# husheng876/pytorch_nested-unet

Hardware: AMD Instinct MI355X
Metric: images/sec NestedUNet 96x96 bs=16 train (higher is better)
Workload: dtype bf16; 1 GPU; NestedUNet(num_classes=1, in=3, deep_supervision=False) 96x96 per-GPU batch 16, bf16 storage / fp32 accumulate, BCEDiceLoss, SGD(1e-3, 0.9, wd 1e-4), fwd+loss+iou+bwd+sgd per step (BASELINE.json configs[1]); global_batch=16, parallelism=dp1, hip_graph=True

## Files before the change

### include/nunet.h

```cpp
#ifndef NUNET_H
#define NUNET_H

#include <stddef.h>
#include <stdint.h>

#ifdef __cplusplus
extern "C" {
#endif

typedef void* nunet_stream_t;

enum { NUNET_F32 = 0, NUNET_BF16 = 1, NUNET_F16 = 2 };
enum {
  NUNET_OK = 0,
  NUNET_EINVAL = -1,
  NUNET_ELAUNCH = -2,
  NUNET_ENODEV = -3
};

int nunet_version(void);
const char* nunet_last_error(void);

#define NUNET_BN_SUM_REPLICAS 8
#define NUNET_FX_WORDS 2
// ... 260 lines not shown
int nunet_plan_grad_scratch(const nunet_plan* p, int64_t* byte_offset, int64_t* bucket0_floats,
                            int64_t* total_floats);
int nunet_plan_bucket0_wait(nunet_plan* p, nunet_stream_t s);
int nunet_plan_opt_step(nunet_plan* p, float* params, const nunet_optim* opt, void* arena, size_t arena_bytes, float grad_scale,
                        float* grads, nunet_stream_t s);
size_t nunet_plan_grad_sqnorm_ws_bytes(const nunet_plan* p);
int nunet_plan_grad_sqnorm(nunet_plan* p, const void* arena, size_t arena_bytes, double* ws, size_t ws_bytes, nunet_stream_t s);
int nunet_plan_repack(nunet_plan* p, const float* params, void* arena, size_t arena_bytes, nunet_stream_t s);
int nunet_plan_set_multistream(nunet_plan* p, int32_t enable);
enum { NUNET_SCHEDULE_LANES = 0, NUNET_SCHEDULE_LIST = 2 };
int nunet_plan_calibrate(nunet_plan* p, int32_t begin);
int nunet_plan_set_lane_priority(nunet_plan* p, int32_t lowest);
int nunet_plan_reset_lanes(nunet_plan* p);
int nunet_plan_set_schedule(nunet_plan* p, int32_t schedule);
int nunet_plan_set_wgrad_dy(nunet_plan* p, int32_t in_loader);
int64_t nunet_plan_feature(const nunet_plan* p, int32_t i, int32_t j, int32_t* pitch,
                           int32_t* channels);

typedef struct {
  char name[48];
  int32_t launches;
  double ms, flops, bytes;
} nunet_prof_entry;
int nunet_profile_begin(void);
int nunet_profile_end(nunet_prof_entry* out, int32_t max_entries, int32_t* n_out);
typedef struct nunet_graph nunet_graph;
int nunet_graph_begin(nunet_stream_t stream);
int nunet_graph_end(nunet_stream_t stream, nunet_graph** out);
int nunet_graph_launch(nunet_graph* graph, nunet_stream_t stream);
int nunet_graph_info(const nunet_graph* graph, int32_t* nodes, int32_t* edges, int32_t* lanes);
// ... 15 lines not shown
```

### pytorch_nested-unet_amd/_lib.py

```python
import ctypes as C
import os
import subprocess

import torch

_HERE = os.path.dirname(os.path.abspath(__file__))
LIB_PATH = os.environ.get("NUNET_LIB_PATH") or os.path.join(_HERE, "libnunet.so")

F32, BF16, F16 = 0, 1, 2
DTYPES = {"fp32": F32, "float32": F32, "bf16": BF16, "bfloat16": BF16, "fp16": F16, "float16": F16,
          torch.float32: F32, torch.bfloat16: BF16, torch.float16: F16}
TORCH_DTYPE = {F32: torch.float32, BF16: torch.bfloat16, F16: torch.float16}

_vp, _i32, _i64, _u32, _f32, _sz = C.c_void_p, C.c_int32, C.c_int64, C.c_uint32, C.c_float, C.c_size_t
BN_SUM_REPLICAS = 8
FX_WORDS = 2
TF_NONE, TF_BN_RELU, TF_BN_RELU_BWD = 0, 1, 2


def fx_zeros(c, device):
    return torch.zeros(BN_SUM_REPLICAS * 2 * c * FX_WORDS, dtype=torch.int64, device=device)


def fx_decode(buf, c):
# ... 212 lines not shown
    "nunet_plan_backward_phase": (_i32, [_vp, _vp, _vp, _vp, _sz, _vp, _i32, _i32, _vp]),
    "nunet_plan_grad_scratch": (_i32, [_vp, C.POINTER(_i64), C.POINTER(_i64), C.POINTER(_i64)]),
    "nunet_plan_bucket0_wait": (_i32, [_vp, _vp]),
    "nunet_plan_opt_step": (_i32, [_vp, _vp, C.POINTER(Optim), _vp, _sz, _f32, _vp, _vp]),
    "nunet_plan_grad_sqnorm_ws_bytes": (C.c_size_t, [_vp]),
    "nunet_plan_grad_sqnorm": (_i32, [_vp, _vp, _sz, _vp, _sz, _vp]),
    "nunet_plan_repack": (_i32, [_vp, _vp, _vp, _sz, _vp]),
    "nunet_plan_feature": (_i64, [_vp, _i32, _i32, C.POINTER(_i32), C.POINTER(_i32)]),
    "nunet_plan_feature_grad": (_i64, [_vp, _i32, _i32, C.POINTER(_i32), C.POINTER(_i32)]),
    "nunet_plan_block_act1": (_i32, [_vp, _vp, _vp, _sz, _i32, _i32, _vp, _vp]),
    "nunet_plan_census_count": (_i32, [_vp, _i32]),
    "nunet_plan_census_get": (_i32, [_vp, _i32, _i32, C.POINTER(PlanCensusEntry)]),
    "nunet_plan_set_multistream": (_i32, [_vp, _i32]),
    "nunet_plan_set_schedule": (_i32, [_vp, _i32]),
    "nunet_plan_set_wgrad_dy": (_i32, [_vp, _i32]),
    "nunet_plan_calibrate": (_i32, [_vp, _i32]),
    "nunet_plan_set_lane_priority": (_i32, [_vp, _i32]),
    "nunet_plan_reset_lanes": (_i32, [_vp]),
    "nunet_plan_set_lanes": (_i32, [_vp, C.POINTER(_vp), _i32]),
    "nunet_profile_begin": (_i32, []),
    "nunet_profile_end": (_i32, [C.POINTER(ProfEntry), _i32, C.POINTER(_i32)]),
    "nunet_debug_spin": (_i32, [_i32, _i32, _vp]),
    "nunet_debug_stamp": (_i32, [_vp, _vp]),
    "nunet_conv3x3_launch_info": (_i32, [C.POINTER(ConvDesc), C.POINTER(ConvLaunchInfo)]),
    "nunet_conv3x3_wgrad_launch_info": (_i32, [C.POINTER(WgradDesc), C.POINTER(WgradLaunchInfo)]),
    "nunet_conv_kernel_attrs": (_i32, [C.POINTER(ConvDesc), C.POINTER(ConvKernelAttrs)]),
    "nunet_loss_launch_info": (_i32, [_i32, _i32, _i64, _i32, C.POINTER(LossLaunchInfo)]),
    "nunet_graph_begin": (_i32, [_vp]),
    "nunet_graph_end": (_i32, [_vp, C.POINTER(_vp)]),
    "nunet_graph_launch": (_i32, [_vp, _vp]),
# ... 84 lines not shown
```

### pytorch_nested-unet_amd/csrc/common.h

```cpp
#pragma once
#include <hip/hip_runtime.h>
#include <hip/hip_ext.h>
#include <stdint.h>
#include <stdio.h>
#include <stdarg.h>
#include <string.h>
#include <type_traits>

#include "../../include/nunet.h"
#include "../../include/nunet_diag.h"

typedef __bf16 bf16_t;
typedef _Float16 f16_t;

typedef __attribute__((ext_vector_type(4))) float f32x4;
typedef __attribute__((ext_vector_type(16))) float f32x16;
typedef __attribute__((ext_vector_type(8))) __bf16 bf16x8;
typedef __attribute__((ext_vector_type(8))) _Float16 f16x8;
typedef __attribute__((ext_vector_type(4))) short s16x4;
typedef __attribute__((ext_vector_type(4))) uint32_t u32x4;

#define WAVE 64
#define CONV_GROUP_MAX 4

// ... 32 lines not shown
    if (pe0_) hipExtLaunchKernelGGL(kernel, grid, block, shmem, stream, pe0_, pe1_, 0, __VA_ARGS__);            \
    else hipLaunchKernelGGL(kernel, grid, block, shmem, stream, __VA_ARGS__);                                   \
  } while (0)

int nunet_zero_async(void* p, size_t bytes, hipStream_t st);

bool seg_active();
bool seg_wait(hipStream_t st, hipEvent_t ev);
bool seg_record(hipEvent_t ev, hipStream_t st);
void seg_touch(hipStream_t st);

static inline int dtype_size(int dt) { return dt == NUNET_F32 ? 4 : 2; }
static inline int ceil_div(int a, int b) { return (a + b - 1) / b; }
static inline int64_t ceil_div64(int64_t a, int64_t b) { return (a + b - 1) / b; }
static inline size_t align_up(size_t a, size_t b) { return (a + b - 1) / b * b; }

template <typename T> struct Tr;
template <> struct Tr<float> {
  static constexpr int EPV = 4;
  static constexpr int DT = NUNET_F32;
};
template <> struct Tr<bf16_t> {
  static constexpr int EPV = 8;
  static constexpr int DT = NUNET_BF16;
};
template <> struct Tr<f16_t> {
  static constexpr int EPV = 8;
  static constexpr int DT = NUNET_F16;
};

// ... 166 lines not shown
  A = __builtin_fmaf(-B, mean, sc * k1);
}

template <typename T> __device__ __forceinline__ Vec16<T> ld16(const T* p) {
  Vec16<T> v;
  v.raw = *reinterpret_cast<const u32x4*>(p);
  return v;
}
template <typename T> __device__ __forceinline__ void st16(T* p, const Vec16<T>& v) {
  *reinterpret_cast<u32x4*>(p) = v.raw;
}
template <typename T> __device__ __forceinline__ Vec16<T> zero16() {
  Vec16<T> v;
  v.raw = u32x4{0u, 0u, 0u, 0u};
  return v;
}

__device__ __forceinline__ float wave_sum(float v) {
#pragma unroll
  for (int o = 32; o > 0; o >>= 1) v += __shfl_xor(v, o);
  return v;
}

__device__ __forceinline__ double wave_sum_f64(double v) {
#pragma unroll
  for (int o = 32; o > 0; o >>= 1) v += __shfl_xor(v, o);
  return v;
}
__device__ __forceinline__ double block256_sum_f64(double v, double* s_w4) {
  v = wave_sum_f64(v);
// ... 99 lines not shown
```

### pytorch_nested-unet_amd/csrc/elementwise.hip

```cpp
#include <cmath>
#include <stdlib.h>
#include <string.h>

#include "common.h"

static thread_local char g_err[512] = "";
void nunet_set_error(const char* fmt, ...) {
  va_list ap;
  va_start(ap, fmt);
  vsnprintf(g_err, sizeof(g_err), fmt, ap);
  va_end(ap);
}
int nunet_check_launch(const char* what) {
  hipError_t e = hipGetLastError();
  if (e != hipSuccess) {
    nunet_set_error("%s: launch failed: %s", what, hipGetErrorString(e));
    return NUNET_ELAUNCH;
  }
  static int trace = -1;
  if (trace < 0) { const char* t = getenv("NUNET_TRACE_LAUNCH"); trace = t ? atoi(t) : 0; }
  if (trace) {
    fprintf(stderr, "[nunet] %s ... ", what); fflush(stderr);
    e = hipDeviceSynchronize();
    fprintf(stderr, "%s\n", e == hipSuccess ? "ok" : hipGetErrorString(e)); fflush(stderr);
    if (e != hipSuccess) { nunet_set_error("%s: execution failed: %s", what, hipGetErrorString(e)); return NUNET_ELAUNCH; }
  }
  return NUNET_OK;
}
extern "C" const char* nunet_last_error(void) { return g_err; }
extern "C" int nunet_version(void) { return 104; }

static inline int grid_for(int64_t items, int block, int cap = 256 * 16) {
  int64_t g = ceil_div64(items, block);
  if (g > cap) g = cap;
  if (g < 1) g = 1;
  return (int)g;
}

__global__ __launch_bounds__(256) void zero_kernel(u32x4* __restrict__ p16, size_t n16, uint32_t* __restrict__ tail, int ntail) {
  const u32x4 z = {0u, 0u, 0u, 0u};
  for (size_t i = blockIdx.x * (size_t)blockDim.x + threadIdx.x; i < n16; i += (size_t)gridDim.x * blockDim.x) p16[i] = z;
  if (blockIdx.x == 0 && (int)threadIdx.x < ntail) tail[threadIdx.x] = 0u;
}
int nunet_zero_async(void* p, size_t bytes, hipStream_t st) {
  NUNET_REQUIRE(((uintptr_t)p % 16) == 0 && bytes % 4 == 0, "zero: buffer must be 16-byte aligned, size a multiple of 4");
  const size_t n16 = bytes / 16;
  const int ntail = (int)((bytes % 16) / 4);
  NUNET_LAUNCH(zero_kernel, dim3(grid_for((int64_t)n16, 256 * 4, 2048)), dim3(256), 0, st, (u32x4*)p, n16,
                     (uint32_t*)((char*)p + n16 * 16), ntail);
  return nunet_check_launch("zero");
}

template <typename T>
__global__ __launch_bounds__(256) void nchw_to_nhwc_kernel(const float* __restrict__ x, int C, int hw, T* __restrict__ y, int cpad, int gshift) {
  constexpr int EPV = Tr<T>::EPV;
  const int n = blockIdx.y;
  const int groups = 1 << gshift;
  const float* xi = x + (size_t)n * C * hw;
  T* yi = y + (size_t)n * hw * cpad;
  for (int j = blockIdx.x * blockDim.x + threadIdx.x; j < (hw << gshift); j += gridDim.x * blockDim.x) {
    const int pix = j >> gshift, c0 = (j & (groups - 1)) * EPV;
    Vec16<T> v;
#pragma unroll
    for (int e = 0; e < EPV; ++e) v.set(e, c0 + e < C ? xi[(size_t)(c0 + e) * hw + pix] : 0.f);
    st16(yi + (size_t)pix * cpad + c0, v);
  }
}
template <typename T> static int launch_nchw_to_nhwc(const float* x, int N, int C, int H, int W, void* y, int cpad, hipStream_t st) {
  constexpr int EPV = Tr<T>::EPV;
  const int groups = cpad / EPV;
  int gshift = 0;
  while ((1 << gshift) < groups) ++gshift;
  NUNET_REQUIRE(cpad % EPV == 0 && (1 << gshift) == groups && N <= 65535, "nchw_to_nhwc: cpad=%d must be a power-of-two number of 16-byte groups", cpad);
  const long long hw = (long long)H * W;
  NUNET_REQUIRE(hw * groups < (1ll << 31), "nchw_to_nhwc: image too large");
  const int64_t total = (int64_t)N * H * W * cpad;
  ProfScope ps(PC_LAYOUT, 0, (double)total * sizeof(T) + (double)N * C * H * W * 4, st);
  NUNET_LAUNCH((nchw_to_nhwc_kernel<T>), dim3(grid_for(hw * groups, 256, 1024), N), dim3(256), 0, st, x, C, (int)hw, (T*)y, cpad, gshift);
  return nunet_check_launch("nchw_to_nhwc");
}
extern "C" int nunet_nchw_to_nhwc(const float* x, int32_t N, int32_t C, int32_t H, int32_t W, int32_t dtype, void* y, int32_t cpad, nunet_stream_t s) {
  NUNET_REQUIRE(x && y && N > 0 && C > 0 && H > 0 && W > 0 && cpad >= C, "nchw_to_nhwc: bad args");
  return NUNET_DISPATCH(dtype, launch_nchw_to_nhwc, x, N, C, H, W, y, cpad, (hipStream_t)s);
}

__global__ __launch_bounds__(256) void preprocess_u8_kernel(const uint8_t* __restrict__ u, int N, int H, int W, int C,
                                                             const float* __restrict__ mean, const float* __restrict__ stdv,
                                                             const int32_t* __restrict__ aug, float post_scale, float* __restrict__ out) {
  const int64_t total = (int64_t)N * C * H * W;
  for (int64_t i = blockIdx.x * (int64_t)blockDim.x + threadIdx.x; i < total; i += (int64_t)gridDim.x * blockDim.x) {
    const int x = (int)(i % W);
    int64_t t = i / W;
    const int y = (int)(t % H); t /= H;
// ... 1881 lines not shown
```

### pytorch_nested-unet_amd/csrc/plan.hip

```cpp
#include <stdlib.h>
#include <string.h>

#include <initializer_list>
#include <functional>
#include <algorithm>

#include <map>
#include <string>
#include <vector>
#include <stdarg.h>

#include "common.h"

static const int NBF[5] = {32, 64, 128, 256, 512};

#define MAXENT 40
#define HEAD_SLABS 256
struct PackEnt { long long src, wf, wd; int cout, cin, cinpad; };
struct PackTab { int n; int ntiles; PackEnt e[MAXENT]; int tile0[MAXENT + 1]; };
struct UnpackEnt { long long src, dst; int cout, cin, cinpad, taps, nvec, nslab; };
struct UnpackTab { int n; int accumulate; UnpackEnt e[MAXENT]; };

constexpr int TILE_LD = 32 * 9 + 1;
struct Tile { int e, co0, ci0, cw, rw; };
// ... 177 lines not shown
struct UpdP { float* params; const float* scratch; float* grads; float gscale; };

template <typename O>
__device__ __forceinline__ void step_elem(const UpdP& u, const O& o, bool live, float gs, long long idx, float g) {
  g *= gs;
  if (u.grads) u.grads[idx] = g;
  if (live) u.params[idx] = opt_elem(o, u.params[idx], g, idx);
}

static void pack_tiles(PackTab& tab) {
  int nt = 0;
  for (int i = 0; i < tab.n; ++i) { tab.tile0[i] = nt; nt += ((tab.e[i].cout + 31) / 32) * ((tab.e[i].cinpad + 31) / 32); }
  tab.tile0[tab.n] = nt; tab.ntiles = nt;
}

template <typename T> static int launch_pack(const float* params, void* arena_t, const PackTab& tab, hipStream_t st) {
  double pb = 0;
  for (int i = 0; i < tab.n; ++i) pb += 9.0 * tab.e[i].cout * tab.e[i].cin * (4 + (tab.e[i].wd >= 0 ? 2 : 1) * sizeof(T));
  ProfScope ps(PC_PACK, 0, pb, st);
  NUNET_LAUNCH((pack_kernel<T>), dim3(tab.ntiles), dim3(256), 0, st, params, (T*)arena_t, tab);
  return nunet_check_launch("pack_weights");
}

extern "C" int nunet_pack_weights(const float* w, int32_t cout, int32_t cin, int32_t cin_pad, int32_t dtype, void* wf, void* wd, nunet_stream_t s) {
  NUNET_REQUIRE(w && wf && cout > 0 && cin > 0 && cin_pad >= cin, "pack_weights: bad args");
  NUNET_REQUIRE(dtype >= 0 && dtype <= 2, "pack_weights: bad dtype");
  PackTab tab; memset(&tab, 0, sizeof(tab));
  tab.n = 1;
  const int es = dtype_size(dtype);
  char* base = (wd && (char*)wd < (char*)wf) ? (char*)wd : (char*)wf;
  NUNET_REQUIRE(((char*)wf - base) % es == 0 && (!wd || ((char*)wd - base) % es == 0), "pack_weights: wf/wd misaligned");
  tab.e[0].src = 0;
  tab.e[0].wf = ((char*)wf - base) / es;
  tab.e[0].wd = wd ? ((char*)wd - base) / es : -1;
  tab.e[0].cout = cout; tab.e[0].cin = cin; tab.e[0].cinpad = cin_pad;
  pack_tiles(tab);
// ... 35 lines not shown
  bool bn2_in_head;
};
struct Head { long long w_off, b_off, gs; int slot; int acc, bnr_block; };
#define NUNET_MAX_BLOCKS 15
#define NUNET_MAX_HEADS 4

#define NLANES 10
struct PlanRt {
  hipStream_t lanes[NLANES];
  bool lanes_ok;
  std::vector<hipEvent_t> events[2];
  size_t events_used[2];
  int multistream;
  int schedule;
  int wgrad_dy;
  bool lanes_external;
  std::vector<hipStream_t> cap_streams;
  size_t cap_next;
  unsigned long long* stamps;
  int lane_low_priority;
  int calibrating;
  std::map<std::string, float> op_cost[2];
  hipStream_t seg_lanes[3];
  std::vector<hipStream_t> seg_owned;
  struct Sched* open_sched;
  std::vector<hipEvent_t> b0_events;
  std::vector<std::string> stamp_labels[2];
  std::vector<nunet_plan_census_entry> census[2];
};
void graph_tag_tail(hipStream_t st, int lane);
// ... 225 lines not shown
    ue.src = P->heads[k].gs; ue.dst = P->heads[k].w_off; ue.cout = cfg->num_classes; ue.cin = NBF[0]; ue.cinpad = NBF[0]; ue.taps = 1; ue.nvec = 1; ue.nslab = HEAD_SLABS;
  }
  PlanRt* rt = new PlanRt();
  rt->lanes_ok = true;
  rt->lanes_external = false;
  rt->cap_next = 0;
  rt->stamps = nullptr;
  rt->calibrating = 0;
  rt->lane_low_priority = 1;
  rt->open_sched = nullptr;
  rt->seg_lanes[0] = rt->seg_lanes[1] = rt->seg_lanes[2] = nullptr;
  rt->events_used[0] = rt->events_used[1] = 0;
  { const char* e = getenv("NUNET_MULTISTREAM"); rt->multistream = e ? atoi(e) : 1; }
  rt->schedule = NUNET_SCHEDULE_LANES;
  { const char* e = getenv("NUNET_WGRAD_DY"); rt->wgrad_dy = e ? (atoi(e) != 0) : 0; }
  for (int l = 0; l < NLANES; ++l) {
    rt->lanes[l] = nullptr;
    if (hipStreamCreateWithFlags(&rt->lanes[l], hipStreamNonBlocking) != hipSuccess) { rt->lanes_ok = false; (void)hipGetLastError(); }
  }
  P->rt = rt;
  return P;
}

extern "C" nunet_plan* nunet_plan_create(const nunet_plan_cfg* cfg) { return plan_create_impl(cfg, 0); }

extern "C" nunet_plan* nunet_plan_create_pruned(const nunet_plan_cfg* cfg, int32_t depth) {
  if (!cfg) { nunet_set_error("plan_create_pruned: null cfg"); return nullptr; }
  if (depth < 1 || depth > 4) { nunet_set_error("plan_create_pruned: depth %d is not one of 1..4 (the heads final1..final4, archs1.py:105-109)", (int)depth); return nullptr; }
  if (cfg->unet) { nunet_set_error("plan_create_pruned: the plain UNet has no nested sub-networks to prune to"); return nullptr; }
  if (!cfg->deep_supervision) { nunet_set_error("plan_create_pruned: pruning to depth %d needs deep_supervision = 1 (a model without it has no final%d head)", (int)depth, (int)depth); return nullptr; }
// ... 55 lines not shown
  do {                          \
    int rc_ = (expr);           \
    if (rc_ != NUNET_OK) return rc_; \
  } while (0)

static inline char* AB(void* arena, size_t off) { return (char*)arena + off; }

#define NRES 512
enum {
  R_X = 0, R_GX = 25,
  R_BLK = 50,
  R_IMG = 230, R_LOGITS = 231, R_DLOGITS = 232,
  R_WP = 233,
  R_GSW = 240, R_GSV = 280,
  R_GSH = 310,
  R_LVL = 330,
  R_SK = 470
};
enum { B_Y1 = 0, B_Y2, B_UP, B_PIN, B_ST1, B_ST2, B_STRIDE = 8 };
enum { L_DY0 = 0, L_DY1, L_DA1, L_GUP, L_GPIN, L_STRIDE = 8 };
static_assert(B_ST2 < B_STRIDE && L_GPIN < L_STRIDE && R_X + 5 * 5 <= R_GX && R_GX + 5 * 5 <= R_BLK && R_BLK + NUNET_MAX_BLOCKS * B_STRIDE <= R_IMG &&
              R_IMG < R_LOGITS && R_LOGITS < R_DLOGITS && R_DLOGITS < R_WP && R_WP + 5 <= R_GSW && R_GSW + 2 * NUNET_MAX_BLOCKS <= R_GSV &&
              R_GSV + 2 * NUNET_MAX_BLOCKS <= R_GSH && R_GSH + NUNET_MAX_HEADS <= R_LVL && R_LVL + NUNET_MAX_BLOCKS * L_STRIDE <= R_SK &&
              R_SK + NUNET_MAX_BLOCKS <= NRES, "resource-id ranges overlap at this capacity");

struct Sched {
  hipStream_t main_s;
  hipStream_t lane_s[NLANES];
  hipEvent_t lane_tail[NLANES];
  bool multi, capturing, failed;
  bool used[NLANES];
  PlanRt* rt;
  std::vector<hipEvent_t>* pool;
  size_t* pool_used;
  struct Res { hipEvent_t w_ev; hipStream_t w_st; hipEvent_t r_ev[NLANES]; hipStream_t r_st[NLANES]; };
  Res res[NRES];
  int cur_lane; int nreads, nwrites; int reads[16], writes[16];
  hipEvent_t fork_ev;
// ... 382 lines not shown
}
static void set_wgrad_bn_bwd(nunet_wgrad_desc& w, const BnView& v) {
  w.d_tf = NUNET_TF_BN_RELU_BWD; w.d_y = v.y; w.d_py = v.C; w.d_sums = v.fx;
  w.d_mean_invstd = v.mean_invstd; w.d_gamma = v.gamma; w.d_beta = v.beta;
}
static int set_splitk(nunet_conv_desc& d, const nunet_plan* P, void* arena, int k) {
  const Node& n = P->exec[k];
  if (n.sk_floats > 0) { d.splitk_ws = (float*)AB(arena, n.sk); d.splitk_ws_floats = n.sk_floats; }
  return n.sk_floats > 0 ? R_SK + k : -1;
}

#define ARENA_CHECK(what) \
  NUNET_REQUIRE(arena_bytes >= P->total, what ": arena of %zu bytes, nunet_plan_arena_bytes() = %zu", (size_t)arena_bytes, P->total); \
  NUNET_REQUIRE(((uintptr_t)arena & 255) == 0, what ": arena must be 256-byte aligned")

extern "C" int nunet_plan_forward(nunet_plan* P, const float* params, float* bnbuf, int64_t* nbt, const float* input, void* arena, size_t arena_bytes, float* logits, int32_t training_flags, nunet_stream_t s) {
  const int32_t training = training_flags & 1;
  const bool staged = (training_flags & 4) != 0;
  NUNET_REQUIRE(P, "plan_forward: null plan");
  NUNET_REQUIRE(!(training && P->depth), "plan_forward: training mode on a plan pruned to depth %d (nunet_plan_create_pruned): it runs eval forwards only", P->depth);
  NUNET_REQUIRE(params && (input || staged) && arena && logits, "plan_forward: null pointer");
  ARENA_CHECK("plan_forward");
  NUNET_REQUIRE(bnbuf, "plan_forward: bnbuf (running stats) required");
  hipStream_t st = (hipStream_t)s;
  const nunet_plan_cfg& c = P->cfg;
  const int dt = c.dtype, es = P->es;
  char* wpack = AB(arena, P->off_wpack);
  if (training) CK(nunet_zero_async(AB(arena, P->off_fx), 2 * fx_region_bytes(P), st));
  if (!staged) CK(nunet_nchw_to_nhwc(input, c.N, c.input_channels, c.H, c.W, dt, AB(arena, P->off_img), 32, (nunet_stream_t)st));

  Sched S; S.init(P, st, 0);
  const bool skip_pack = (training_flags & 2) != 0;
  if (!skip_pack) {
    S.name("pack");
    S.add(0, 0, 15.f, {}, {R_WP + 0, R_WP + 1, R_WP + 2, R_WP + 3, R_WP + 4}, [=](hipStream_t ls) {
      return NUNET_DISPATCH(dt, launch_pack, params, wpack, P->ptab, ls);
    });
  }
  for (int k = 0; k < (int)P->exec.size(); ++k) {
    const Node& n = P->exec[k];
    const int i = n.i, f = NBF[i], H = P->hl[i], W = P->wl[i];
    const int lane = lane_of(P, n), rb = R_BLK + k * B_STRIDE;
    const Cat in = block_in(P, arena, k, false);
    const BnView bn1 = bn_view(P, arena, params, k, 0, 0), bn2 = bn_view(P, arena, params, k, 1, 0);
    if (n.up_slot >= 0) {
      const Buf x = slot_of(P, arena, false, i + 1, n.up_slot);
      S.name("B%d%d.upF", n.i, n.j);
      S.add(lane, 0, 7.f, {x.r}, {in.r[4]}, [=](hipStream_t ls) {
// ... 284 lines not shown
#pragma unroll 4
    for (int sl = part; sl < en.ks; sl += 4) {
      const f32x4 v = *reinterpret_cast<const f32x4*>(q + (size_t)sl * en.stride);
      a[0] += v[0]; a[1] += v[1]; a[2] += v[2]; a[3] += v[3];
    }
  }
  s_p[part][el] = a;
  __syncthreads();
  if (part == 0 && i < en.n4) {
    f32x4 r = s_p[0][el];
#pragma unroll
    for (int q = 1; q < 4; ++q) { const f32x4 v = s_p[q][el]; r[0] += v[0]; r[1] += v[1]; r[2] += v[2]; r[3] += v[3]; }
    *reinterpret_cast<f32x4*>(gs + en.dst + i * 4) = r;
  }
}
static int launch_reduce(nunet_plan* P, void* arena, int k_lo, int k_hi, hipStream_t st) {
  RedTab tab; tab.n = 0; tab.nblocks = 0;
  double bytes = 0;
  for (int k = k_hi; k >= k_lo; --k)
    for (int cv = 1; cv >= 0; --cv) {
      const ConvL& c = cv ? P->exec[k].c2 : P->exec[k].c1;
      if (c.ks <= 1) continue;
      RedEnt& en = tab.e[tab.n++];
      en.slab = c.slab; en.dst = c.gs; en.stride = 9LL * c.cout * c.cinpad; en.n4 = en.stride / 4; en.ks = c.ks; en.blk0 = tab.nblocks;
      tab.nblocks += (int)((en.n4 + 63) / 64);
      bytes += (double)en.stride * 4 * (c.ks + 1);
    }
  if (tab.n == 0) return NUNET_OK;
  ProfScope ps(PC_UNPACK, 0, bytes, st);
  NUNET_LAUNCH(reduce_kernel, dim3(tab.nblocks), dim3(256), 0, st, (const float*)AB(arena, P->off_slab), (float*)AB(arena, P->off_gs), tab);
  return nunet_check_launch("wgrad slab reduce");
}

extern "C" int nunet_plan_backward_phase(nunet_plan* P, const float* params, const float* dlogits, void* arena, size_t arena_bytes, float* grads, int32_t accumulate, int32_t phases, nunet_stream_t s) {
  if (P) REFUSE_PRUNED("plan_backward");
  if (phases != 3 && phases != 7 && phases != 4 && phases != (1 | 8) && phases != (2 | 16)) {
    nunet_set_error("plan_backward: phases %d is not one of 3, 7, 4, 1|8 = 9, 2|16 = 18", (int)phases); return NUNET_EINVAL;
// ... 41 lines not shown

  for (int k = k_hi; k >= k_lo; --k) {
    const Node& n = P->exec[k];
    const int i = n.i, f = NBF[i], H = P->hl[i], W = P->wl[i];
    const int lane = lane_of(P, n), wlane = 5 + lane, rb = R_BLK + k * B_STRIDE, rl = R_LVL + k * L_STRIDE;
    const Buf gxo = slot_of(P, arena, true, i, n.out_slot);
    if (spin_us > 0 && k == k_split - 1 && (phases & 2)) {
      const int us = spin_us;
      S.name("spin");
      S.add(lane, 0, 0.f, {gxo.r}, {gxo.r}, [=](hipStream_t ls) { return nunet_debug_spin(us, 1, (nunet_stream_t)ls); });
    }
    const ConvL& L1 = n.c1; const ConvL& L2 = n.c2;
    const BnView bn1 = bn_view(P, arena, params, k, 0, 1), bn2 = bn_view(P, arena, params, k, 1, 1);
    const Buf dy2 = {AB(arena, n.dy[0]), rl + L_DY0}, dy1 = {AB(arena, n.dy[1]), rl + L_DY1}, da1 = {AB(arena, n.da1), rl + L_DA1};
    const bool has_dgrad1 = !(i == 0 && n.in_prefix == 0);
    const bool dy2_in_wgrad = rt->wgrad_dy != 0, dy1_in_wgrad = rt->wgrad_dy != 0 || !has_dgrad1;

    if (!n.bn2_in_head) {
      nunet_bn_bwd_desc b2; memset(&b2, 0, sizeof(b2));
      b2.dtype = dt; b2.N = c.N; b2.H = H; b2.W = W; b2.C = f;
      b2.da = gxo.p; b2.PDA = P->PX[i]; set_bn(b2, bn2);
      S.name("B%d%d.bnR2", n.i, n.j);
      S.add(lane, 0, 9.f, {gxo.r, bn2.r_y}, {bn2.r_fx}, [=](hipStream_t ls) { return nunet_bn_relu_bwd_reduce(&b2, ls); });
    }

    {
      nunet_conv_desc d; memset(&d, 0, sizeof(d));
      d.dtype = dt; d.N = c.N; d.H = H; d.W = W;
      d.src0 = gxo.p; d.C0 = f; d.P0 = P->PX[i];
      set_tf_bn_bwd(d, bn2);
      d.tf_store = dy2_in_wgrad ? nullptr : dy2.p; d.tf_ps = f;
      d.wpack = wpack + (size_t)L2.wd * es;
      d.dst0 = da1.p; d.D0 = f; d.Q0 = f;
      d.bn_y = bn1.y; d.bn_py = f; d.bn_mean_invstd = bn1.mean_invstd;
      d.bn_gamma = bn1.gamma; d.bn_beta = bn1.beta; d.bn_sums = bn1.fx;
      const int rsk = set_splitk(d, P, arena, k);
      S.name("B%d%d.dgrad2", n.i, n.j);
      S.add_conv(lane, {gxo.r, bn2.r_y, bn1.r_y, R_WP + i}, {dy2_in_wgrad ? -1 : dy2.r, da1.r, bn2.r_fx, bn1.r_fx, rsk}, d);
    }
    if (has_dgrad1) {
      const Cat g = block_in(P, arena, k, true);
      nunet_conv_desc d; memset(&d, 0, sizeof(d));
      d.dtype = dt; d.N = c.N; d.H = H; d.W = W;
      d.src0 = da1.p; d.C0 = f; d.P0 = f;
      set_tf_bn_bwd(d, bn1);
      d.tf_store = dy1_in_wgrad ? nullptr : dy1.p; d.tf_ps = f;
      d.wpack = wpack + (size_t)L1.wd * es;
      d.dst0 = g.p[0]; d.D0 = g.c[0]; d.Q0 = g.pitch[0];
      d.dst1 = g.p[1]; d.D1 = g.c[1]; d.Q1 = g.pitch[1];
      if (n.in_prefix > 0) { d.acc_slot_w = f; d.acc0_mask = n.acc0_mask; }
      const int rsk = set_splitk(d, P, arena, k);
      S.name("B%d%d.dgrad1", n.i, n.j);
      S.add_conv(lane, {da1.r, bn1.r_y, bn1.r_fx, R_WP + i}, {dy1_in_wgrad ? -1 : dy1.r, g.r[0], g.r[1], g.r[2], g.r[3], g.r[4], rsk}, d);
      if (n.in_prefix == 0) {
        const Buf x = slot_of(P, arena, false, i - 1, 0), gx = slot_of(P, arena, true, i - 1, 0);
        S.name("B%d%d.poolB", n.i, n.j);
        S.add(lane, 0, 8.f, {g.r[0], x.r}, {gx.r}, [=](hipStream_t ls) {
          return nunet_maxpool2x2_bwd(dt, c.N, P->hl[i - 1], P->wl[i - 1], NBF[i - 1], x.p, P->PX[i - 1], g.p[0], NBF[i - 1], gx.p, P->PX[i - 1], n.acc_pool, ls);
        });
      } else {
        const Buf gx = slot_of(P, arena, true, i + 1, n.up_slot);
        S.name("B%d%d.upB", n.i, n.j);
        S.add(lane, 0, 11.f, {g.r[4]}, {gx.r}, [=](hipStream_t ls) {
          return nunet_upsample2x_bwd(dt, c.N, P->hl[i + 1], P->wl[i + 1], NBF[i + 1], g.p[1], NBF[i + 1], gx.p, P->PX[i + 1], n.acc_up, ls);
        });
      }
    }
    {
      const Cat in = block_in(P, arena, k, false);
      nunet_wgrad_desc w1, w2; memset(&w1, 0, sizeof(w1)); memset(&w2, 0, sizeof(w2));
      w1.dtype = w2.dtype = dt; w1.N = w2.N = c.N; w1.H = w2.H = H; w1.W = w2.W = W;
      w2.src0 = bn1.y; w2.C0 = f; w2.P0 = f;
      w2.x_tf = NUNET_TF_BN_RELU; w2.x_mean_invstd = bn1.mean_invstd; w2.x_gamma = bn1.gamma; w2.x_beta = bn1.beta;
      set_src(w1, in);
      w1.dy = dy1.p; w2.dy = dy2.p; w1.Cout = w2.Cout = f; w1.PY = w2.PY = f;
      if (dy2_in_wgrad) { w2.dy = gxo.p; w2.PY = P->PX[i]; set_wgrad_bn_bwd(w2, bn2); }
      if (dy1_in_wgrad) {
        w1.dy = da1.p; w1.PY = f; set_wgrad_bn_bwd(w1, bn1);
        if (!has_dgrad1) { w1.d_dbias = bn1.gv; w1.d_dgamma = bn1.gv + bn1.C; w1.d_dbeta = bn1.gv + 2 * bn1.C; }
      }
      w1.dw = L1.ks > 1 ? slabs + L1.slab : gsr + L1.gs; w1.slab_stride = 9LL * L1.cout * L1.cinpad; w1.max_slabs = L1.ks; w1.target_wgs = L1.wg_target;
      w2.dw = L2.ks > 1 ? slabs + L2.slab : gsr + L2.gs; w2.slab_stride = 9LL * L2.cout * L2.cinpad; w2.max_slabs = L2.ks; w2.target_wgs = L2.wg_target;
      w1.dw_floats = (int64_t)L1.ks * w1.slab_stride; w2.dw_floats = (int64_t)L2.ks * w2.slab_stride;
      const int alg_cin = (i == 0 && n.in_prefix == 0) ? c.input_channels : 0;
      S.name("B%d%d.wgrad", n.i, n.j);
      S.census_wgrad(w1, w2);
      int wl = wlane, r_gate = -1;
      if (!P->cfg.unet && n.j > 0 && n.i + n.j == 4 && n.i <= 2 && (phases & 3) == 3 && !S.list) { wl = 4; r_gate = R_GX + 3 * 5 + 1; }
      const float wcost = 8.f + (float)(2.0 * 9 * ((double)L1.cinpad + L2.cinpad) * f * (double)c.N * H * W / 3.5e8);
      const int rd[12] = {bn1.r_y, dy2_in_wgrad ? gxo.r : dy2.r, dy2_in_wgrad ? bn2.r_y : -1, dy2_in_wgrad ? bn2.r_fx : -1,
                          dy1_in_wgrad ? da1.r : dy1.r, dy1_in_wgrad ? bn1.r_fx : -1, in.r[0], in.r[1], in.r[2], in.r[3], in.r[4], r_gate};
      const int wr[3] = {R_GSW + 2 * k, R_GSW + 2 * k + 1, has_dgrad1 ? -1 : bn1.r_fx};
      S.add_v(wl, 1, wcost, rd, 12, wr, 3,
            [=](hipStream_t ls) {
              g_prof_alg_cin = alg_cin; int r = nunet_conv3x3_wgrad_pair(&w1, &w2, ls); g_prof_alg_cin = 0;
              return r ? r : launch_reduce(P, arena, k, k, ls);
            });
    }
  }
  int rc = S.run();
  if (leave_open && rc == NUNET_OK && !S.failed) {
// ... 138 lines not shown
  ARENA_CHECK("plan_block_act1");
  const int k = block_at(P, i, j);
  NUNET_REQUIRE(k >= 0, "plan_block_act1: the plan has no block (%d, %d)", (int)i, (int)j);
  const nunet_plan_cfg& c = P->cfg;
  const Node& n = P->exec[k];
  const BnView bn1 = bn_view(P, arena, params, k, 0, 0);
  nunet_bn_fwd_desc b; memset(&b, 0, sizeof(b));
  b.dtype = c.dtype; b.N = c.N; b.H = P->hl[i]; b.W = P->wl[i]; b.C = NBF[i];
  b.y = bn1.y; b.PY = NBF[i]; b.conv_bias = params + n.c1.b_off; b.stats = bn1.fx;
  b.gamma = bn1.gamma; b.beta = bn1.beta;
  b.save_mean_invstd = bn1.mean_invstd; b.training = 1; b.momentum = 0.1f; b.eps = 1e-5f;
  b.a = out; b.PA = NBF[i];
  return nunet_bn_relu_fwd(&b, s);
}

extern "C" int nunet_plan_set_multistream(nunet_plan* P, int32_t enable) {
  NUNET_REQUIRE(P, "plan_set_multistream: null plan");
  rt_of(P)->multistream = enable;
  return NUNET_OK;
}
```

### pytorch_nested-unet_amd/engine.py

```python
import ctypes as C

import torch

from . import _lib as L


class Plan:
    def __init__(self, n, h, w, cin, ncls, ds, dtype, unet, device, depth=None):
        lib = L.lib()
        cfg = L.PlanCfg(n, h, w, cin, ncls, 1 if ds else 0, dtype, 1 if unet else 0)
        if depth is None:
            self.handle = lib.nunet_plan_create(C.byref(cfg))
            if not self.handle:
                raise L.NunetError("nunet_plan_create: " + lib.nunet_last_error().decode())
        else:
            self.handle = lib.nunet_plan_create_pruned(C.byref(cfg), int(depth))
            if not self.handle:
                raise L.NunetError("nunet_plan_create_pruned: " + lib.nunet_last_error().decode())
        self.depth = depth
        self.n, self.h, self.w, self.ncls, self.dtype = n, h, w, ncls, dtype
        self.heads = lib.nunet_plan_num_heads(self.handle)
        self.nparams = lib.nunet_plan_param_count(self.handle)
        self.nbnbuf = lib.nunet_plan_bnbuf_count(self.handle)
        self.nbn = lib.nunet_plan_bn_layers(self.handle)
# ... 17 lines not shown
        return self._slot(L.lib().nunet_plan_feature_grad, i, j)

    def block_act1(self, i, j):
        if self.params is None or not self.trained_forward:
            raise L.NunetError("block_act1 needs a training-mode forward of this plan through its Engine first")
        pitch, ch = C.c_int32(), C.c_int32()
        if L.lib().nunet_plan_feature(self.handle, i, j, C.byref(pitch), C.byref(ch)) < 0:
            raise L.NunetError("no block (%d, %d)" % (i, j))
        out = torch.empty((self.n, self.h >> i, self.w >> i, ch.value), dtype=L.TORCH_DTYPE[self.dtype], device=self.arena.device)
        L.check(L.lib().nunet_plan_block_act1(self.handle, L.ptr(self.params), L.ptr(self.arena), L.nbytes(self.arena), i, j,
                                              L.ptr(out), L.stream()), "nunet_plan_block_act1")
        return out

    def set_wgrad_dy(self, in_loader):
        L.check(L.lib().nunet_plan_set_wgrad_dy(self.handle, 1 if in_loader else 0), "nunet_plan_set_wgrad_dy")

    def census(self, backward):
        lib, out = L.lib(), []
        for k in range(lib.nunet_plan_census_count(self.handle, int(backward))):
            e = L.PlanCensusEntry()
            L.check(lib.nunet_plan_census_get(self.handle, int(backward), k, C.byref(e)), "nunet_plan_census_get")
            out.append(e)
        return out

    def _slot(self, query, i, j):
        pitch, ch = C.c_int32(), C.c_int32()
        off = query(self.handle, i, j, C.byref(pitch), C.byref(ch))
        if off < 0:
            raise L.NunetError("no feature x%d_%d" % (i, j))
        es = 4 if self.dtype == L.F32 else 2
# ... 114 lines not shown
```

Before: 9805 images/sec.

## Fuse step prologue kernels and add optional split tail wgrad scheduling

Adds a single step_prologue kernel that uses block-index role dispatch to do weight packing, NCHW-to-NHWC input layout and the zeroing of the BN-sum buffer in one launch. It is on by default and replaces up to three launches at the start of a training step. Separately adds an opt-in tail_split mode, off by default, that issues the first block's conv2 weight gradient ahead of dgrad2 on its own lane. The fused kernel removes launch and graph-node overhead but serialises the packing work inside one grid and changes scheduling dependencies.

```diff
diff --git a/include/nunet.h b/include/nunet.h
--- a/include/nunet.h
+++ b/include/nunet.h
@@ -298,6 +298,7 @@
 int nunet_plan_reset_lanes(nunet_plan* p);
 int nunet_plan_set_schedule(nunet_plan* p, int32_t schedule);
 int nunet_plan_set_wgrad_dy(nunet_plan* p, int32_t in_loader);
+int nunet_plan_set_tail_split(nunet_plan* p, int32_t on);
 int64_t nunet_plan_feature(const nunet_plan* p, int32_t i, int32_t j, int32_t* pitch,
                            int32_t* channels);
 
diff --git a/pytorch_nested-unet_amd/_lib.py b/pytorch_nested-unet_amd/_lib.py
--- a/pytorch_nested-unet_amd/_lib.py
+++ b/pytorch_nested-unet_amd/_lib.py
@@ -250,6 +250,7 @@
     "nunet_plan_set_multistream": (_i32, [_vp, _i32]),
     "nunet_plan_set_schedule": (_i32, [_vp, _i32]),
     "nunet_plan_set_wgrad_dy": (_i32, [_vp, _i32]),
+    "nunet_plan_set_tail_split": (_i32, [_vp, _i32]),
     "nunet_plan_calibrate": (_i32, [_vp, _i32]),
     "nunet_plan_set_lane_priority": (_i32, [_vp, _i32]),
     "nunet_plan_reset_lanes": (_i32, [_vp]),
diff --git a/pytorch_nested-unet_amd/csrc/common.h b/pytorch_nested-unet_amd/csrc/common.h
--- a/pytorch_nested-unet_amd/csrc/common.h
+++ b/pytorch_nested-unet_amd/csrc/common.h
@@ -70,6 +70,14 @@
 static inline int ceil_div(int a, int b) { return (a + b - 1) / b; }
 static inline int64_t ceil_div64(int64_t a, int64_t b) { return (a + b - 1) / b; }
 static inline size_t align_up(size_t a, size_t b) { return (a + b - 1) / b * b; }
+static inline int grid_for(int64_t items, int block, int cap = 256 * 16) {
+  int64_t g = ceil_div64(items, block);
+  if (g > cap) g = cap;
+  if (g < 1) g = 1;
+  return (int)g;
+}
+static inline int zero_grid(size_t n16) { return grid_for((int64_t)n16, 256 * 4, 2048); }
+static inline int layout_grid(long long hw, int groups) { return grid_for(hw * groups, 256, 1024); }
 
 template <typename T> struct Tr;
 template <> struct Tr<float> {
@@ -266,6 +274,25 @@
   Vec16<T> v;
   v.raw = u32x4{0u, 0u, 0u, 0u};
   return v;
+}
+
+__device__ __forceinline__ void zero_block(u32x4* __restrict__ p16, size_t n16, int bx, int gx) {
+  const u32x4 z = {0u, 0u, 0u, 0u};
+  for (size_t i = bx * (size_t)blockDim.x + threadIdx.x; i < n16; i += (size_t)gx * blockDim.x) p16[i] = z;
+}
+template <typename T>
+__device__ __forceinline__ void nchw_to_nhwc_block(const float* __restrict__ x, int C, int hw, T* __restrict__ y, int cpad, int gshift, int bx, int gx, int n) {
+  constexpr int EPV = Tr<T>::EPV;
+  const int groups = 1 << gshift;
+  const float* xi = x + (size_t)n * C * hw;
+  T* yi = y + (size_t)n * hw * cpad;
+  for (int j = bx * blockDim.x + threadIdx.x; j < (hw << gshift); j += gx * blockDim.x) {
+    const int pix = j >> gshift, c0 = (j & (groups - 1)) * EPV;
+    Vec16<T> v;
+#pragma unroll
+    for (int e = 0; e < EPV; ++e) v.set(e, c0 + e < C ? xi[(size_t)(c0 + e) * hw + pix] : 0.f);
+    st16(yi + (size_t)pix * cpad + c0, v);
+  }
 }
 
 __device__ __forceinline__ float wave_sum(float v) {
diff --git a/pytorch_nested-unet_amd/csrc/elementwise.hip b/pytorch_nested-unet_amd/csrc/elementwise.hip
--- a/pytorch_nested-unet_amd/csrc/elementwise.hip
+++ b/pytorch_nested-unet_amd/csrc/elementwise.hip
@@ -30,41 +30,22 @@
 extern "C" const char* nunet_last_error(void) { return g_err; }
 extern "C" int nunet_version(void) { return 104; }
 
-static inline int grid_for(int64_t items, int block, int cap = 256 * 16) {
-  int64_t g = ceil_div64(items, block);
-  if (g > cap) g = cap;
-  if (g < 1) g = 1;
-  return (int)g;
-}
-
 __global__ __launch_bounds__(256) void zero_kernel(u32x4* __restrict__ p16, size_t n16, uint32_t* __restrict__ tail, int ntail) {
-  const u32x4 z = {0u, 0u, 0u, 0u};
-  for (size_t i = blockIdx.x * (size_t)blockDim.x + threadIdx.x; i < n16; i += (size_t)gridDim.x * blockDim.x) p16[i] = z;
+  zero_block(p16, n16, blockIdx.x, gridDim.x);
   if (blockIdx.x == 0 && (int)threadIdx.x < ntail) tail[threadIdx.x] = 0u;
 }
 int nunet_zero_async(void* p, size_t bytes, hipStream_t st) {
   NUNET_REQUIRE(((uintptr_t)p % 16) == 0 && bytes % 4 == 0, "zero: buffer must be 16-byte aligned, size a multiple of 4");
   const size_t n16 = bytes / 16;
   const int ntail = (int)((bytes % 16) / 4);
-  NUNET_LAUNCH(zero_kernel, dim3(grid_for((int64_t)n16, 256 * 4, 2048)), dim3(256), 0, st, (u32x4*)p, n16,
+  NUNET_LAUNCH(zero_kernel, dim3(zero_grid(n16)), dim3(256), 0, st, (u32x4*)p, n16,
                      (uint32_t*)((char*)p + n16 * 16), ntail);
   return nunet_check_launch("zero");
 }
 
 template <typename T>
 __global__ __launch_bounds__(256) void nchw_to_nhwc_kernel(const float* __restrict__ x, int C, int hw, T* __restrict__ y, int cpad, int gshift) {
-  constexpr int EPV = Tr<T>::EPV;
-  const int n = blockIdx.y;
-  const int groups = 1 << gshift;
-  const float* xi = x + (size_t)n * C * hw;
-  T* yi = y + (size_t)n * hw * cpad;
-  for (int j = blockIdx.x * blockDim.x + threadIdx.x; j < (hw << gshift); j += gridDim.x * blockDim.x) {
-    const int pix = j >> gshift, c0 = (j & (groups - 1)) * EPV;
-    Vec16<T> v;
-#pragma unroll
-    for (int e = 0; e < EPV; ++e) v.set(e, c0 + e < C ? xi[(size_t)(c0 + e) * hw + pix] : 0.f);
-    st16(yi + (size_t)pix * cpad + c0, v);
-  }
+  nchw_to_nhwc_block(x, C, hw, y, cpad, gshift, blockIdx.x, gridDim.x, blockIdx.y);
 }
 template <typename T> static int launch_nchw_to_nhwc(const float* x, int N, int C, int H, int W, void* y, int cpad, hipStream_t st) {
   constexpr int EPV = Tr<T>::EPV;
@@ -76,7 +57,7 @@
   NUNET_REQUIRE(hw * groups < (1ll << 31), "nchw_to_nhwc: image too large");
   const int64_t total = (int64_t)N * H * W * cpad;
   ProfScope ps(PC_LAYOUT, 0, (double)total * sizeof(T) + (double)N * C * H * W * 4, st);
-  NUNET_LAUNCH((nchw_to_nhwc_kernel<T>), dim3(grid_for(hw * groups, 256, 1024), N), dim3(256), 0, st, x, C, (int)hw, (T*)y, cpad, gshift);
+  NUNET_LAUNCH((nchw_to_nhwc_kernel<T>), dim3(layout_grid(hw, groups), N), dim3(256), 0, st, x, C, (int)hw, (T*)y, cpad, gshift);
   return nunet_check_launch("nchw_to_nhwc");
 }
 extern "C" int nunet_nchw_to_nhwc(const float* x, int32_t N, int32_t C, int32_t H, int32_t W, int32_t dtype, void* y, int32_t cpad, nunet_stream_t s) {
diff --git a/pytorch_nested-unet_amd/csrc/plan.hip b/pytorch_nested-unet_amd/csrc/plan.hip
--- a/pytorch_nested-unet_amd/csrc/plan.hip
+++ b/pytorch_nested-unet_amd/csrc/plan.hip
@@ -215,12 +215,46 @@
   tab.tile0[tab.n] = nt; tab.ntiles = nt;
 }
 
+static double pack_bytes(const PackTab& tab, size_t es) {
+  double pb = 0;
+  for (int i = 0; i < tab.n; ++i) pb += 9.0 * tab.e[i].cout * tab.e[i].cin * (4 + (tab.e[i].wd >= 0 ? 2 : 1) * es);
+  return pb;
+}
 template <typename T> static int launch_pack(const float* params, void* arena_t, const PackTab& tab, hipStream_t st) {
-  double pb = 0;
-  for (int i = 0; i < tab.n; ++i) pb += 9.0 * tab.e[i].cout * tab.e[i].cin * (4 + (tab.e[i].wd >= 0 ? 2 : 1) * sizeof(T));
-  ProfScope ps(PC_PACK, 0, pb, st);
+  ProfScope ps(PC_PACK, 0, pack_bytes(tab, sizeof(T)), st);
   NUNET_LAUNCH((pack_kernel<T>), dim3(tab.ntiles), dim3(256), 0, st, params, (T*)arena_t, tab);
   return nunet_check_launch("pack_weights");
+}
+
+struct PrologueRoles {
+  int npack;
+  int nlayout, lgx; const float* x; void* img; int C, hw, cpad, gshift;
+  int nzero; u32x4* z16; size_t n16;
+};
+template <typename T>
+__global__ __launch_bounds__(256) void step_prologue_kernel(const float* __restrict__ params, T* __restrict__ arena, PackTab tab, PrologueRoles r) {
+  __shared__ float s_t[32][TILE_LD];
+  int b = blockIdx.x;
+  if (b < r.npack) {
+    const Tile t = tile_of(tab, b);
+    const PackEnt en = tab.e[t.e];
+    load_oihw_tile(s_t, params + en.src, en, t);
+    __syncthreads();
+    store_packed_tile(s_t, arena, en, t);
+    return;
+  }
+  b -= r.npack;
+  if (b < r.nlayout) {
+    const int n = b / r.lgx;
+    nchw_to_nhwc_block(r.x, r.C, r.hw, (T*)r.img, r.cpad, r.gshift, b - n * r.lgx, r.lgx, n);
+    return;
+  }
+  zero_block(r.z16, r.n16, b - r.nlayout, r.nzero);
+}
+template <typename T> static int launch_step_prologue(const float* params, void* arena_t, const PackTab& tab, PrologueRoles r, double bytes, hipStream_t st) {
+  ProfScope ps(PC_PACK, 0, bytes, st);
+  NUNET_LAUNCH((step_prologue_kernel<T>), dim3(r.npack + r.nlayout + r.nzero), dim3(256), 0, st, params, (T*)arena_t, tab, r);
+  return nunet_check_launch("step_prologue");
 }
 
 extern "C" int nunet_pack_weights(const float* w, int32_t cout, int32_t cin, int32_t cin_pad, int32_t dtype, void* wf, void* wd, nunet_stream_t s) {
@@ -286,6 +320,8 @@
   int multistream;
   int schedule;
   int wgrad_dy;
+  int tail_split;
+  int step_prologue;
   bool lanes_external;
   std::vector<hipStream_t> cap_streams;
   size_t cap_next;
@@ -541,6 +577,8 @@
   { const char* e = getenv("NUNET_MULTISTREAM"); rt->multistream = e ? atoi(e) : 1; }
   rt->schedule = NUNET_SCHEDULE_LANES;
   { const char* e = getenv("NUNET_WGRAD_DY"); rt->wgrad_dy = e ? (atoi(e) != 0) : 0; }
+  { const char* e = getenv("NUNET_TAIL_SPLIT"); rt->tail_split = e ? (atoi(e) != 0) : 0; }
+  { const char* e = getenv("NUNET_STEP_PROLOGUE"); rt->step_prologue = e ? (atoi(e) != 0) : 1; }
   for (int l = 0; l < NLANES; ++l) {
     rt->lanes[l] = nullptr;
     if (hipStreamCreateWithFlags(&rt->lanes[l], hipStreamNonBlocking) != hipSuccess) { rt->lanes_ok = false; (void)hipGetLastError(); }
@@ -626,6 +664,7 @@
   R_WP = 233,
   R_GSW = 240, R_GSV = 280,
   R_GSH = 310,
+  R_GV2 = 314,
   R_LVL = 330,
   R_SK = 470
 };
@@ -633,7 +672,7 @@
 enum { L_DY0 = 0, L_DY1, L_DA1, L_GUP, L_GPIN, L_STRIDE = 8 };
 static_assert(B_ST2 < B_STRIDE && L_GPIN < L_STRIDE && R_X + 5 * 5 <= R_GX && R_GX + 5 * 5 <= R_BLK && R_BLK + NUNET_MAX_BLOCKS * B_STRIDE <= R_IMG &&
               R_IMG < R_LOGITS && R_LOGITS < R_DLOGITS && R_DLOGITS < R_WP && R_WP + 5 <= R_GSW && R_GSW + 2 * NUNET_MAX_BLOCKS <= R_GSV &&
-              R_GSV + 2 * NUNET_MAX_BLOCKS <= R_GSH && R_GSH + NUNET_MAX_HEADS <= R_LVL && R_LVL + NUNET_MAX_BLOCKS * L_STRIDE <= R_SK &&
+              R_GSV + 2 * NUNET_MAX_BLOCKS <= R_GSH && R_GSH + NUNET_MAX_HEADS <= R_GV2 && R_GV2 < R_LVL && R_LVL + NUNET_MAX_BLOCKS * L_STRIDE <= R_SK &&
               R_SK + NUNET_MAX_BLOCKS <= NRES, "resource-id ranges overlap at this capacity");
 
 struct Sched {
@@ -1046,6 +1085,29 @@
   NUNET_REQUIRE(arena_bytes >= P->total, what ": arena of %zu bytes, nunet_plan_arena_bytes() = %zu", (size_t)arena_bytes, P->total); \
   NUNET_REQUIRE(((uintptr_t)arena & 255) == 0, what ": arena must be 256-byte aligned")
 
+template <typename T>
+static int plan_step_prologue(nunet_plan* P, const float* params, const float* input, void* arena, bool zero, bool layout, bool pack, hipStream_t st) {
+  constexpr int EPV = Tr<T>::EPV;
+  const nunet_plan_cfg& c = P->cfg;
+  PrologueRoles r; memset(&r, 0, sizeof(r));
+  double bytes = 0;
+  if (pack) { r.npack = P->ptab.ntiles; bytes += pack_bytes(P->ptab, sizeof(T)); }
+  if (layout) {
+    const int groups = 32 / EPV;
+    while ((1 << r.gshift) < groups) ++r.gshift;
+    const long long hw = (long long)c.H * c.W;
+    NUNET_REQUIRE(hw * groups < (1ll << 31) && (long long)c.N * layout_grid(hw, groups) < (1ll << 30), "plan_forward: image too large");
+    r.lgx = layout_grid(hw, groups); r.nlayout = r.lgx * c.N;
+    r.x = input; r.img = AB(arena, P->off_img); r.C = c.input_channels; r.hw = (int)hw; r.cpad = 32;
+    bytes += (double)c.N * hw * (32.0 * sizeof(T) + 4.0 * c.input_channels);
+  }
+  if (zero) {
+    r.z16 = (u32x4*)AB(arena, P->off_fx); r.n16 = 2 * fx_region_bytes(P) / 16; r.nzero = zero_grid(r.n16);
+    bytes += 16.0 * r.n16;
+  }
+  return launch_step_prologue<T>(params, AB(arena, P->off_wpack), P->ptab, r, bytes, st);
+}
+
 extern "C" int nunet_plan_forward(nunet_plan* P, const float* params, float* bnbuf, int64_t* nbt, const float* input, void* arena, size_t arena_bytes, float* logits, int32_t training_flags, nunet_stream_t s) {
   const int32_t training = training_flags & 1;
   const bool staged = (training_flags & 4) != 0;
@@ -1058,12 +1120,17 @@
   const nunet_plan_cfg& c = P->cfg;
   const int dt = c.dtype, es = P->es;
   char* wpack = AB(arena, P->off_wpack);
-  if (training) CK(nunet_zero_async(AB(arena, P->off_fx), 2 * fx_region_bytes(P), st));
-  if (!staged) CK(nunet_nchw_to_nhwc(input, c.N, c.input_channels, c.H, c.W, dt, AB(arena, P->off_img), 32, (nunet_stream_t)st));
+  const bool skip_pack = (training_flags & 2) != 0;
+  const size_t zero_bytes = 2 * fx_region_bytes(P);
+  const bool fused = rt_of(P)->step_prologue && (training != 0) + !staged + !skip_pack >= 2 && zero_bytes % 16 == 0;
+  if (fused) CK(NUNET_DISPATCH(dt, plan_step_prologue, P, params, input, arena, training != 0, !staged, !skip_pack, st));
+  else {
+    if (training) CK(nunet_zero_async(AB(arena, P->off_fx), zero_bytes, st));
+    if (!staged) CK(nunet_nchw_to_nhwc(input, c.N, c.input_channels, c.H, c.W, dt, AB(arena, P->off_img), 32, (nunet_stream_t)st));
+  }
 
   Sched S; S.init(P, st, 0);
-  const bool skip_pack = (training_flags & 2) != 0;
-  if (!skip_pack) {
+  if (!skip_pack && !fused) {
     S.name("pack");
     S.add(0, 0, 15.f, {}, {R_WP + 0, R_WP + 1, R_WP + 2, R_WP + 3, R_WP + 4}, [=](hipStream_t ls) {
       return NUNET_DISPATCH(dt, launch_pack, params, wpack, P->ptab, ls);
@@ -1378,13 +1445,13 @@
     *reinterpret_cast<f32x4*>(gs + en.dst + i * 4) = r;
   }
 }
-static int launch_reduce(nunet_plan* P, void* arena, int k_lo, int k_hi, hipStream_t st) {
+static int launch_reduce(nunet_plan* P, void* arena, int k_lo, int k_hi, hipStream_t st, int layers = 3) {
   RedTab tab; tab.n = 0; tab.nblocks = 0;
   double bytes = 0;
   for (int k = k_hi; k >= k_lo; --k)
     for (int cv = 1; cv >= 0; --cv) {
       const ConvL& c = cv ? P->exec[k].c2 : P->exec[k].c1;
-      if (c.ks <= 1) continue;
+      if (c.ks <= 1 || !(layers >> cv & 1)) continue;
       RedEnt& en = tab.e[tab.n++];
       en.slab = c.slab; en.dst = c.gs; en.stride = 9LL * c.cout * c.cinpad; en.n4 = en.stride / 4; en.ks = c.ks; en.blk0 = tab.nblocks;
       tab.nblocks += (int)((en.n4 + 63) / 64);
@@ -1456,7 +1523,8 @@
     const BnView bn1 = bn_view(P, arena, params, k, 0, 1), bn2 = bn_view(P, arena, params, k, 1, 1);
     const Buf dy2 = {AB(arena, n.dy[0]), rl + L_DY0}, dy1 = {AB(arena, n.dy[1]), rl + L_DY1}, da1 = {AB(arena, n.da1), rl + L_DA1};
     const bool has_dgrad1 = !(i == 0 && n.in_prefix == 0);
-    const bool dy2_in_wgrad = rt->wgrad_dy != 0, dy1_in_wgrad = rt->wgrad_dy != 0 || !has_dgrad1;
+    const bool split_tail = rt->tail_split != 0 && !has_dgrad1 && rt->wgrad_dy == 0;
+    const bool dy2_in_wgrad = rt->wgrad_dy != 0 || split_tail, dy1_in_wgrad = rt->wgrad_dy != 0 || !has_dgrad1;
 
     if (!n.bn2_in_head) {
       nunet_bn_bwd_desc b2; memset(&b2, 0, sizeof(b2));
@@ -1464,6 +1532,30 @@
       b2.da = gxo.p; b2.PDA = P->PX[i]; set_bn(b2, bn2);
       S.name("B%d%d.bnR2", n.i, n.j);
       S.add(lane, 0, 9.f, {gxo.r, bn2.r_y}, {bn2.r_fx}, [=](hipStream_t ls) { return nunet_bn_relu_bwd_reduce(&b2, ls); });
+    }
+
+    const Cat in = block_in(P, arena, k, false);
+    nunet_wgrad_desc w1, w2; memset(&w1, 0, sizeof(w1)); memset(&w2, 0, sizeof(w2));
+    {
+      w1.dtype = w2.dtype = dt; w1.N = w2.N = c.N; w1.H = w2.H = H; w1.W = w2.W = W;
+      w2.src0 = bn1.y; w2.C0 = f; w2.P0 = f;
+      w2.x_tf = NUNET_TF_BN_RELU; w2.x_mean_invstd = bn1.mean_invstd; w2.x_gamma = bn1.gamma; w2.x_beta = bn1.beta;
+      set_src(w1, in);
+      w1.dy = dy1.p; w2.dy = dy2.p; w1.Cout = w2.Cout = f; w1.PY = w2.PY = f;
+      if (dy2_in_wgrad) { w2.dy = gxo.p; w2.PY = P->PX[i]; set_wgrad_bn_bwd(w2, bn2); }
+      if (dy1_in_wgrad) {
+        w1.dy = da1.p; w1.PY = f; set_wgrad_bn_bwd(w1, bn1);
+        if (!has_dgrad1) { w1.d_dbias = bn1.gv; w1.d_dgamma = bn1.gv + bn1.C; w1.d_dbeta = bn1.gv + 2 * bn1.C; }
+      }
+      w1.dw = L1.ks > 1 ? slabs + L1.slab : gsr + L1.gs; w1.slab_stride = 9LL * L1.cout * L1.cinpad; w1.max_slabs = L1.ks; w1.target_wgs = L1.wg_target;
+      w2.dw = L2.ks > 1 ? slabs + L2.slab : gsr + L2.gs; w2.slab_stride = 9LL * L2.cout * L2.cinpad; w2.max_slabs = L2.ks; w2.target_wgs = L2.wg_target;
+      w1.dw_floats = (int64_t)L1.ks * w1.slab_stride; w2.dw_floats = (int64_t)L2.ks * w2.slab_stride;
+    }
+    const auto wgrad_cost = [&](int cinpads) { return 8.f + (float)(2.0 * 9 * (double)cinpads * f * (double)c.N * H * W / 3.5e8); };
+    if (split_tail) {
+      S.name("B%d%d.wgrad2", n.i, n.j);
+      S.add(S.list ? wlane : 4, 1, wgrad_cost(L2.cinpad), {bn1.r_y, gxo.r, bn2.r_y, bn2.r_fx}, {R_GSW + 2 * k + 1},
+            [=](hipStream_t ls) { const int r = nunet_conv3x3_wgrad(&w2, ls); return r ? r : launch_reduce(P, arena, k, k, ls, 2); });
     }
 
     {
@@ -1478,7 +1570,8 @@
       d.bn_gamma = bn1.gamma; d.bn_beta = bn1.beta; d.bn_sums = bn1.fx;
       const int rsk = set_splitk(d, P, arena, k);
       S.name("B%d%d.dgrad2", n.i, n.j);
-      S.add_conv(lane, {gxo.r, bn2.r_y, bn1.r_y, R_WP + i}, {dy2_in_wgrad ? -1 : dy2.r, da1.r, bn2.r_fx, bn1.r_fx, rsk}, d);
+      S.add_conv(lane, {gxo.r, bn2.r_y, bn1.r_y, R_WP + i, split_tail ? bn2.r_fx : -1},
+                 {dy2_in_wgrad ? -1 : dy2.r, da1.r, split_tail ? R_GV2 : bn2.r_fx, bn1.r_fx, rsk}, d);
     }
     if (has_dgrad1) {
       const Cat g = block_in(P, arena, k, true);
@@ -1509,24 +1602,16 @@
       }
     }
     {
-      const Cat in = block_in(P, arena, k, false);
-      nunet_wgrad_desc w1, w2; memset(&w1, 0, sizeof(w1)); memset(&w2, 0, sizeof(w2));
-      w1.dtype = w2.dtype = dt; w1.N = w2.N = c.N; w1.H = w2.H = H; w1.W = w2.W = W;
-      w2.src0 = bn1.y; w2.C0 = f; w2.P0 = f;
-      w2.x_tf = NUNET_TF_BN_RELU; w2.x_mean_invstd = bn1.mean_invstd; w2.x_gamma = bn1.gamma; w2.x_beta = bn1.beta;
-      set_src(w1, in);
-      w1.dy = dy1.p; w2.dy = dy2.p; w1.Cout = w2.Cout = f; w1.PY = w2.PY = f;
-      if (dy2_in_wgrad) { w2.dy = gxo.p; w2.PY = P->PX[i]; set_wgrad_bn_bwd(w2, bn2); }
-      if (dy1_in_wgrad) {
-        w1.dy = da1.p; w1.PY = f; set_wgrad_bn_bwd(w1, bn1);
-        if (!has_dgrad1) { w1.d_dbias = bn1.gv; w1.d_dgamma = bn1.gv + bn1.C; w1.d_dbeta = bn1.gv + 2 * bn1.C; }
-      }
-      w1.dw = L1.ks > 1 ? slabs + L1.slab : gsr + L1.gs; w1.slab_stride = 9LL * L1.cout * L1.cinpad; w1.max_slabs = L1.ks; w1.target_wgs = L1.wg_target;
-      w2.dw = L2.ks > 1 ? slabs + L2.slab : gsr + L2.gs; w2.slab_stride = 9LL * L2.cout * L2.cinpad; w2.max_slabs = L2.ks; w2.target_wgs = L2.wg_target;
-      w1.dw_floats = (int64_t)L1.ks * w1.slab_stride; w2.dw_floats = (int64_t)L2.ks * w2.slab_stride;
       const int alg_cin = (i == 0 && n.in_prefix == 0) ? c.input_channels : 0;
       S.name("B%d%d.wgrad", n.i, n.j);
       S.census_wgrad(w1, w2);
+      if (split_tail) {
+        S.add(wlane, 1, wgrad_cost(L1.cinpad), {da1.r, bn1.r_y, bn1.r_fx, in.r[0]}, {R_GSW + 2 * k, bn1.r_fx}, [=](hipStream_t ls) {
+          g_prof_alg_cin = alg_cin; const int r = nunet_conv3x3_wgrad(&w1, ls); g_prof_alg_cin = 0;
+          return r ? r : launch_reduce(P, arena, k, k, ls, 1);
+        });
+        continue;
+      }
       int wl = wlane, r_gate = -1;
       if (!P->cfg.unet && n.j > 0 && n.i + n.j == 4 && n.i <= 2 && (phases & 3) == 3 && !S.list) { wl = 4; r_gate = R_GX + 3 * 5 + 1; }
       const float wcost = 8.f + (float)(2.0 * 9 * ((double)L1.cinpad + L2.cinpad) * f * (double)c.N * H * W / 3.5e8);
@@ -1695,6 +1780,15 @@
   return nunet_bn_relu_fwd(&b, s);
 }
 
+extern "C" int nunet_plan_set_tail_split(nunet_plan* P, int32_t on) {
+  NUNET_REQUIRE(P, "plan_set_tail_split: null plan");
+  REFUSE_PRUNED("plan_set_tail_split");
+  NUNET_REQUIRE(on == 0 || on == 1, "plan_set_tail_split: %d is neither 0 (the block's weight gradients as one pair behind dgrad2) nor 1 (conv2's ahead of it)", on);
+  NUNET_REQUIRE(!rt_of(P)->open_sched, "plan_set_tail_split: a backward pass is open (nunet_plan_backward_phase 1|8)");
+  rt_of(P)->tail_split = on;
+  return NUNET_OK;
+}
+
 extern "C" int nunet_plan_set_multistream(nunet_plan* P, int32_t enable) {
   NUNET_REQUIRE(P, "plan_set_multistream: null plan");
   rt_of(P)->multistream = enable;
diff --git a/pytorch_nested-unet_amd/engine.py b/pytorch_nested-unet_amd/engine.py
--- a/pytorch_nested-unet_amd/engine.py
+++ b/pytorch_nested-unet_amd/engine.py
@@ -55,6 +55,9 @@
 
     def set_wgrad_dy(self, in_loader):
         L.check(L.lib().nunet_plan_set_wgrad_dy(self.handle, 1 if in_loader else 0), "nunet_plan_set_wgrad_dy")
+
+    def set_tail_split(self, on):
+        L.check(L.lib().nunet_plan_set_tail_split(self.handle, 1 if on else 0), "nunet_plan_set_tail_split")
 
     def census(self, backward):
         lib, out = L.lib(), []
```

After: 9883 images/sec (median of 6 runs). About the same (+0.8%).
